# microsoft/M3P

Hardware: AMD Instinct MI355X
Metric: pre-train samples/sec (whole node), 12L/768d seq=128+36 (higher is better)
Workload: dtype bf16; 1 GPU; cfg2: 12L/768d/12h, 36 regions + 128 tokens, V=250002, 19 MLM targets/seq + ITM BCE, dropout 0.10, adam_inverse_sqrt + clip 5; per_gpu_batch=256, global_batch=256, seq_len=164, parallelism=dp1, prewarm_steps=36

## Files before the change

include/m3p_hip.h:

```cpp
#ifndef M3P_HIP_H
#define M3P_HIP_H

#include <stddef.h>
#include <stdint.h>

#ifdef __cplusplus
extern "C" {
#endif

#define M3P_API __attribute__((visibility("default")))

#define M3P_OK 0
#define M3P_EINVAL (-1)
#define M3P_ENOTIMPL (-2)
#define M3P_ENOMEM (-3)

M3P_API const char* m3p_version(void);


enum {
  M3P_EPI_NONE = 0,
  M3P_EPI_BIAS = 1,
  M3P_EPI_BIAS_GELU = 2,
  M3P_EPI_BIAS_DROP_RES = 3,
// ... 96 lines not shown
M3P_API int m3p_attn_causal_fwd(const void* qkv, int ld_qkv, void* ctx, float* lse, int B, int T, int H, int dh,
                                uint32_t seed, uint32_t thresh24, float inv_keep, void* stream);
M3P_API int m3p_attn_causal_bwd(const void* qkv, int ld_qkv, const void* dctx, const float* lse, void* dqkv, int ld_dqkv,
                                int B, int T, int H, int dh, float qscale, uint32_t seed, uint32_t thresh24,
                                float inv_keep, void* stream);


M3P_API int m3p_cast_f32_bf16(const float* src, void* dst, long long n, void* stream);

M3P_API int m3p_embed_assemble_fwd(const int64_t* tok, const void* emb_bf16, const float* pos,
                                   const void* img_proj, const float* loc, const float* w_loc,
                                   const float* b_loc, const float* g_img, const float* be_img,
                                   const float* g_emb, const float* be_emb, const int32_t* totlen,
                                   void* h, void* z, float* mean_emb, float* rstd_emb, void* e,
                                   float* mean_img, float* rstd_img, int B, int T, int R, int d,
                                   uint32_t seed_img, uint32_t seed_emb, uint32_t thresh24, float inv_keep,
                                   const void* img_rows, void* stream);

M3P_API int m3p_embed_image_rows_fwd(const void* img_proj, const float* loc, const float* w_loc, const float* b_loc,
                                     const float* g_img, const float* be_img, void* e, float* mean_img,
                                     float* rstd_img, void* img_rows, int B, int R, int d, uint32_t seed_img,
                                     uint32_t thresh24, float inv_keep, void* stream);

M3P_API int m3p_embed_assemble_bwd(const void* dh, const void* z, const float* mean_emb, const float* rstd_emb,
                                   const float* g_emb, const void* e, const float* mean_img,
                                   const float* rstd_img, const float* g_img, const int64_t* tok,
                                   const int32_t* totlen, const float* loc, void* dz_scratch, void* de,
                                   float* d_g_emb, float* d_be_emb, float* d_pos, float* d_emb,
                                   void* d_tok_rows, float* d_g_img, float* d_be_img, float* d_b_img, float* d_b_loc,
                                   float* d_w_loc, int B, int T, int R, int d, int pad_index,
                                   uint32_t seed_img, uint32_t seed_emb, uint32_t thresh24, float inv_keep,
                                   int phase, void* stream);


M3P_API int m3p_gather_rows(const void* src, const int32_t* idx, void* dst, int n, int d, void* stream);
M3P_API int m3p_place_rows(const void* src, const int32_t* inv, void* dst, int rows, int d, int n, uint32_t fill_bits,
                           void* stream);
M3P_API int m3p_scatter_add_rows(const void* src, const int32_t* idx, void* dst, int n, int d, void* stream);
M3P_API int m3p_scatter_add_token_rows(const void* rows, int ld_rows, const int64_t* ids, float* dst, int n, int d,
                                       int pad_index, void* stream);

M3P_API int m3p_itm_score_fwd(const void* pre, const float* w2, const float* b2, float* pooled, float* scores, int B,
                              int d, void* stream);
M3P_API int m3p_itm_score_bwd(const float* dscores, const float* pooled, const float* w2, void* dpre16, void* dpreT16,
                              int ldt, float* db1, float* dw2, float* db2, int B, int d, void* stream);

M3P_API int m3p_ce_fwd_bwd(void* logits, int ld, int n_rows, int V, const int64_t* target, float* row_loss,
                           float* loss_sum, float loss_scale, float grad_scale, void* stream);

M3P_API int m3p_ce_lse_from_blocks(const void* stats, int n_blocks, int n_rows, const void* logits, int ld, const int64_t* target,
                                   float* row_loss, float* row_lse, void* scratch, void* stream);
M3P_API int m3p_ce_bwd_colsum(void* logits, int ld, int n_rows, int V, const int64_t* target, const float* row_lse,
                              float grad_scale, float* colsum, void* workspace, size_t workspace_bytes, void* stream);
M3P_API size_t m3p_ce_colsum_workspace_bytes(int ld, int n_rows);
M3P_API int m3p_ce_fwd_bwd_colsum(void* logits, int ld, int n_rows, int V, const int64_t* target, float* row_loss,
                                  float* row_lse, float grad_scale, float* colsum, void* workspace,
                                  size_t workspace_bytes, void* stream);

M3P_API int m3p_ce_shift_target(const void* h, const void* emb, const float* bias, const int64_t* target, float* row_t, void* row_ref,
                                int n_rows, int d, void* stream);
M3P_API int m3p_ce_shift_rows(const void* stats, int n_blocks, int n_rows, float grad_scale, float* row_loss, float* row_s,
                              float* row_q, void* scratch, void* stream);
M3P_API int m3p_ce_shift_colsum(const void* e, int ld, int n_rows, const float* row_s, float* colsum, void* workspace,
                                size_t workspace_bytes, void* stream);
M3P_API int m3p_ce_shift_scale_rows(const void* h, const float* row_s, const float* g, void* out, int n_rows, int d, void* stream);
M3P_API int m3p_ce_shift_target_rows(const void* h, const int64_t* target, const float* row_q, const float* g, float* demb, float* dbias,
// ... 90 lines not shown
```

m3p_amd/csrc/embed.hip:

```cpp
#include "common.hpp"
#include <hip/amd_detail/amd_hip_unsafe_atomics.h>

namespace {

constexpr int EMB_BWD_BLOCKS = 512;

constexpr float kEps = 1e-12f;

template <int NI>
__device__ __forceinline__ void row_ln(const f32x4 (&v)[NI], int nchunk, int lane, float inv_d, float& mu, float& rs) {
  float s = 0.f;
#pragma unroll
  for (int i = 0; i < NI; ++i) s += (v[i][0] + v[i][1]) + (v[i][2] + v[i][3]);
  mu = wave_sum(s) * inv_d;
  float q = 0.f;
#pragma unroll
  for (int i = 0; i < NI; ++i) {
    if (lane + 64 * i < nchunk) {
      const f32x4 t = v[i] - mu;
      q += (t[0] * t[0] + t[1] * t[1]) + (t[2] * t[2] + t[3] * t[3]);
    }
  }
  rs = 1.0f / sqrtf(wave_sum(q) * inv_d + kEps);
}
// ... 284 lines not shown
        Vec4<bf16>::store(a.de + ri * d + 4 * c, ob);
        acc_e[i] += ob;
#pragma unroll
        for (int k = 0; k < 5; ++k) acc_w[k][i] += ob * lc[k];
      }
    }
  }
  block_reduce_atomic<NI>(red, acc_g, a.d_g_img, d, lane, wib);
  block_reduce_atomic<NI>(red, acc_b, a.d_be_img, d, lane, wib);
#pragma unroll
  for (int i = 0; i < NI; ++i)
#pragma unroll
    for (int j = 0; j < 4; ++j) red[wib][4 * (lane + 64 * i) + j] = acc_e[i][j];
  __syncthreads();
  for (int c = threadIdx.x; c < d; c += blockDim.x) {
    const float v = (red[0][c] + red[1][c]) + (red[2][c] + red[3][c]);
    unsafeAtomicAdd(a.d_b_img + c, v);
    unsafeAtomicAdd(a.d_b_loc + c, v);
  }
  __syncthreads();
#pragma unroll
  for (int k = 0; k < 5; ++k) {
#pragma unroll
    for (int i = 0; i < NI; ++i)
#pragma unroll
      for (int j = 0; j < 4; ++j) red[wib][4 * (lane + 64 * i) + j] = acc_w[k][i][j];
    __syncthreads();
    for (int c = threadIdx.x; c < d; c += blockDim.x)
      unsafeAtomicAdd(a.d_w_loc + (size_t)c * 5 + k, (red[0][c] + red[1][c]) + (red[2][c] + red[3][c]));
    __syncthreads();
  }
}

__global__ __launch_bounds__(256) void cast_f32_bf16_kernel(const float* __restrict__ src, bf16* __restrict__ dst, size_t n4) {
  for (size_t i = (size_t)blockIdx.x * blockDim.x + threadIdx.x; i < n4; i += (size_t)gridDim.x * blockDim.x)
    Vec4<bf16>::store(dst + 4 * i, Vec4<float>::load(src + 4 * i));
}

inline int ni_of(int d) { return (d + 255) / 256; }

int launch_embed_fwd(const EmbedFwdArgs& a, void* stream);
}

extern "C" {

int m3p_cast_f32_bf16(const float* src, void* dst, long long n, void* stream) {
  if (n <= 0 || (n % 4) != 0 || ((uintptr_t)src & 15) || ((uintptr_t)dst & 7)) return M3P_EINVAL;
  const size_t n4 = (size_t)n / 4;
  const int blocks = (int)((n4 + 255) / 256 < 4096 ? (n4 + 255) / 256 : 4096);
  hipLaunchKernelGGL(cast_f32_bf16_kernel, dim3(blocks), dim3(256), 0, (hipStream_t)stream, src, (bf16*)dst, n4);
  M3P_CHECK_LAUNCH();
  return M3P_OK;
}

int m3p_embed_assemble_fwd(const int64_t* tok, const void* emb_bf16, const float* pos, const void* img_proj,
                           const float* loc, const float* w_loc, const float* b_loc, const float* g_img,
                           const float* be_img, const float* g_emb, const float* be_emb, const int32_t* totlen,
                           void* h, void* z, float* mean_emb, float* rstd_emb, void* e, float* mean_img,
                           float* rstd_img, int B, int T, int R, int d, uint32_t seed_img, uint32_t seed_emb,
                           uint32_t thresh24, float inv_keep, const void* img_rows, void* stream) {
  if (B <= 0 || T < 0 || R < 0 || d <= 0 || (d % 4) != 0 || d > 1024) return M3P_EINVAL;
  if (img_rows && ((uintptr_t)img_rows & 7)) return M3P_EINVAL;
  EmbedFwdArgs a = {tok, (const bf16*)emb_bf16, pos, (const bf16*)img_proj, loc, w_loc, b_loc, g_img, be_img, g_emb, be_emb,
                    totlen, (bf16*)h, (bf16*)z, mean_emb, rstd_emb, (bf16*)e, mean_img, rstd_img, B, T, R, d,
                    seed_img, seed_emb, thresh24, inv_keep, (bf16*)const_cast<void*>(img_rows), img_rows ? 2 : 0};
  return launch_embed_fwd(a, stream);
}

int m3p_embed_image_rows_fwd(const void* img_proj, const float* loc, const float* w_loc, const float* b_loc,
                             const float* g_img, const float* be_img, void* e, float* mean_img, float* rstd_img,
                             void* img_rows, int B, int R, int d, uint32_t seed_img, uint32_t thresh24, float inv_keep,
                             void* stream) {
  if (B <= 0 || R <= 0 || d <= 0 || (d % 4) != 0 || d > 1024 || !img_rows || ((uintptr_t)img_rows & 7)) return M3P_EINVAL;
  EmbedFwdArgs a = {nullptr, nullptr, nullptr, (const bf16*)img_proj, loc, w_loc, b_loc, g_img, be_img, nullptr, nullptr,
                    nullptr, nullptr, nullptr, nullptr, nullptr, (bf16*)e, mean_img, rstd_img, B, 0, R, d,
                    seed_img, 0u, thresh24, inv_keep, (bf16*)img_rows, 1};
  return launch_embed_fwd(a, stream);
}

}

namespace {
int launch_embed_fwd(const EmbedFwdArgs& a, void* stream) {
  const int B = a.B, T = a.T, R = a.R, d = a.d;
  const int rows = B * (R + T);
  const int blocks = (rows + 3) / 4 < 4096 ? (rows + 3) / 4 : 4096;
  hipStream_t st = (hipStream_t)stream;
  switch (ni_of(d)) {
    case 1: hipLaunchKernelGGL(embed_fwd_kernel<1>, dim3(blocks), dim3(256), 0, st, a); break;
    case 2: hipLaunchKernelGGL(embed_fwd_kernel<2>, dim3(blocks), dim3(256), 0, st, a); break;
    case 3: hipLaunchKernelGGL(embed_fwd_kernel<3>, dim3(blocks), dim3(256), 0, st, a); break;
    default: hipLaunchKernelGGL(embed_fwd_kernel<4>, dim3(blocks), dim3(256), 0, st, a); break;
  }
  M3P_CHECK_LAUNCH();
  return M3P_OK;
}
}

extern "C" {

int m3p_embed_assemble_bwd(const void* dh, const void* z, const float* mean_emb, const float* rstd_emb,
                           const float* g_emb, const void* e, const float* mean_img, const float* rstd_img,
                           const float* g_img, const int64_t* tok, const int32_t* totlen, const float* loc,
                           void* dz_scratch, void* de, float* d_g_emb, float* d_be_emb, float* d_pos, float* d_emb,
                           void* d_tok_rows, float* d_g_img, float* d_be_img, float* d_b_img, float* d_b_loc, float* d_w_loc,
                           int B, int T, int R, int d, int pad_index, uint32_t seed_img, uint32_t seed_emb,
                           uint32_t thresh24, float inv_keep, int phase, void* stream) {
  if (B <= 0 || T < 0 || R < 0 || d <= 0 || (d % 4) != 0 || d > 1024 || phase < 0 || phase > 2) return M3P_EINVAL;
  int bsplit = 1;
  while (bsplit < 16 && (R + T) * bsplit < EMB_BWD_BLOCKS && B / (4 * bsplit) >= 8) bsplit *= 2;
  EmbedBwdArgs a = {(const bf16*)dh, (const bf16*)z, mean_emb, rstd_emb, g_emb, (const bf16*)e, mean_img, rstd_img, g_img,
                    tok, totlen, loc, (bf16*)dz_scratch, (bf16*)de, d_g_emb, d_be_emb, d_pos, d_emb,
                    (bf16*)d_tok_rows, d_g_img, d_be_img, d_b_img, d_b_loc, d_w_loc, B, T, R, d, pad_index, bsplit,
                    seed_img, seed_emb, thresh24, inv_keep};
  hipStream_t st = (hipStream_t)stream;
  const int S = R + T;
#define M3P_EMB_BWD(NI)                                                                              \
  do {                                                                                               \
    if (phase != 2) hipLaunchKernelGGL(embed_bwd_rows_kernel<NI>, dim3(S* bsplit), dim3(256), 0, st, a);             \
    if (R > 0 && phase != 1) hipLaunchKernelGGL(embed_bwd_img_kernel<NI>, dim3(R* bsplit), dim3(256), 0, st, a);   \
  } while (0)
  switch (ni_of(d)) {
    case 1: M3P_EMB_BWD(1); break;
    case 2: M3P_EMB_BWD(2); break;
    case 3: M3P_EMB_BWD(3); break;
    default: M3P_EMB_BWD(4); break;
  }
#undef M3P_EMB_BWD
  M3P_CHECK_LAUNCH();
  return M3P_OK;
}

}
```

m3p_amd/csrc/glue.hip:

```cpp
#include "common.hpp"

namespace {

__global__ __launch_bounds__(256)
void seq_masks_kernel(const long long* __restrict__ len_a, const long long* __restrict__ len_b, int B, int S,
                      int* __restrict__ totlen, uint8_t* __restrict__ rowmask) {
  const int b = blockIdx.x;
  const int n = (int)(len_a[b] + (len_b ? len_b[b] : 0));
  if (threadIdx.x == 0) totlen[b] = n;
  for (int s = threadIdx.x; s < S; s += blockDim.x) rowmask[(size_t)b * S + s] = (s < n) ? 1 : 0;
}

__global__ __launch_bounds__(1024)
void mask_to_rows_kernel(const uint8_t* __restrict__ mask, int n_mask, int inner, long long s0, long long s1,
                         long long soff, int d, int* __restrict__ rows, int n_rows) {
  __shared__ int wsum[16];
  __shared__ int total_sh;
  const int tid = threadIdx.x, lane = tid & 63, w = tid >> 6;
  const int per = (n_mask + 1023) / 1024;
  const int lo = min(tid * per, n_mask), hi = min(lo + per, n_mask);
  int cnt = 0;
  for (int i = lo; i < hi; ++i) cnt += mask[i] ? 1 : 0;
  int inc = cnt;
#pragma unroll
  for (int o = 1; o < 64; o <<= 1) {
    const int v = __shfl_up(inc, o, 64);
    if (lane >= o) inc += v;
  }
  if (lane == 63) wsum[w] = inc;
  __syncthreads();
  if (tid == 0) {
    int run = 0;
    for (int i = 0; i < 16; ++i) { const int v = wsum[i]; wsum[i] = run; run += v; }
    total_sh = run;
  }
  __syncthreads();
  int pos = wsum[w] + inc - cnt;
  for (int i = lo; i < hi; ++i) {
    if (mask[i]) {
      if (pos < n_rows) {
        const int t = i / inner, b = i - t * inner;
        rows[pos] = (int)((soff + t * s0 + b * s1) / d);
      }
      ++pos;
    }
  }
  for (int k = total_sh + tid; k < n_rows; k += 1024) rows[k] = 0;
}

__global__ __launch_bounds__(256)
void cast_rows_kernel(const float* __restrict__ in, long long s0, long long s1, int n1, int cols,
                      bf16* __restrict__ out, long long nrows) {
  const int cpr = cols >> 2;
  const long long total = nrows * cpr;
  for (long long i = (long long)blockIdx.x * blockDim.x + threadIdx.x; i < total; i += (long long)gridDim.x * blockDim.x) {
    const long long row = i / cpr;
    const int c = (int)(i - row * cpr) * 4;
    const long long i0 = row / n1, i1 = row - i0 * n1;
    const f32x4 v = *reinterpret_cast<const f32x4*>(in + i0 * s0 + i1 * s1 + c);
    *reinterpret_cast<bf16x4*>(out + row * cols + c) = bf16x4{(bf16)v[0], (bf16)v[1], (bf16)v[2], (bf16)v[3]};
  }
}

template <typename TI>
__global__ __launch_bounds__(256)
void scale_to_bf16_kernel(const TI* __restrict__ in, const float* __restrict__ g, bf16* __restrict__ out, long long n4) {
  const float s = g[0];
  for (long long i = (long long)blockIdx.x * blockDim.x + threadIdx.x; i < n4; i += (long long)gridDim.x * blockDim.x) {
    f32x4 v = Vec4<TI>::load(in + 4 * i);
    v *= s;
    Vec4<bf16>::store(out + 4 * i, v);
  }
}

__global__ __launch_bounds__(256)
void axpy_dev_kernel(float* __restrict__ dst, const float* __restrict__ src, const float* __restrict__ g, long long n) {
  const float s = g[0];
  for (long long i = (long long)blockIdx.x * blockDim.x + threadIdx.x; i < n; i += (long long)gridDim.x * blockDim.x)
    dst[i] += s * src[i];
// ... 112 lines not shown
```

m3p_amd/lib.py:

```python
import ctypes as C
import os

import torch

_HERE = os.path.dirname(os.path.abspath(__file__))
LIB_PATH = os.environ.get('M3P_HIP_LIB') or os.path.join(_HERE, 'libm3p_hip.so')

EPI_NONE, EPI_BIAS, EPI_BIAS_GELU, EPI_BIAS_DROP_RES, EPI_RES, EPI_DGELU, EPI_MUL, EPI_MULQ, EPI_BIAS_GELUQ, EPI_BIAS_LSE = range(10)
KERN_NT_SKINNY, KERN_NT_W8, KERN_NT_W8_QUEUE, KERN_NT_W4, KERN_NT_RING, KERN_NT_128 = range(1, 7)
KERN_WGRAD_W4_CHUNKS, KERN_WGRAD_W4_TILES, KERN_WGRAD_RING, KERN_WGRAD_128 = range(10, 14)


class M3PError(RuntimeError):
    pass


class Epilogue(C.Structure):
    _fields_ = [
        ('bias', C.c_void_p), ('aux', C.c_void_p), ('out2', C.c_void_p), ('colsum', C.c_void_p),
        ('ld_aux', C.c_int32), ('ld_out2', C.c_int32), ('scale_cols', C.c_int32), ('scale', C.c_float),
        ('alpha', C.c_float), ('seed', C.c_uint32), ('thresh24', C.c_uint32), ('inv_keep', C.c_float),
        ('descale_a', C.c_void_p), ('descale_b', C.c_void_p),
        ('out8', C.c_void_p), ('scale8', C.c_void_p), ('amax8', C.c_void_p), ('ld_out8', C.c_int32), ('out8_bf8', C.c_int32),
        ('rng_rows', C.c_void_p),
        ('row_ref', C.c_void_p),
    ]


_p, _i, _f, _u32 = C.c_void_p, C.c_int, C.c_float, C.c_uint32

SIGNATURES = {
    'm3p_version': (C.c_char_p, []),
    'm3p_gemm_nt_bf16': (_i, [_p, _i, _p, _i, _p, _i, _i, _i, _i, _i, C.POINTER(Epilogue), _p]),
    'm3p_gemm_nt_fp8': (_i, [_p, _i, _i, _p, _i, _p, _i, _i, _i, _i, _i, C.POINTER(Epilogue), _p]),
    'm3p_quant_fp8': (_i, [_p, _i, _p, _i, _i, _i, _p, _p, _i, _p]),
    'm3p_quant_fp8_batch': (_i, [_p, _i, _i, _p]),
    'm3p_gemm_nt_streamk_f32': (_i, [_p, _i, _p, _i, _p, _i, _i, _i, _i, _f, _p]),
    'm3p_gemm_nn_streamk_f32': (_i, [_p, _i, _p, _i, _i, _p, _i, _i, _i, _i, _f, _p]),
    'm3p_gemm_nn_w4_f32': (_i, [_p, _i, _p, _i, _p, _i, _i, _i, _i, _f, _p, C.c_size_t, _p]),
    'm3p_gemm_wgrad_workspace_bytes': (C.c_size_t, []),
    'm3p_gemm_wgrad_bf16': (_i, [_p, _i, _p, _i, _p, _i, _i, _i, _i, _f, _p, C.c_size_t, _p]),
    'm3p_gemm_wgrad_store_bf16': (_i, [_p, _i, _p, _i, _p, _i, _i, _i, _i, _f, _p, C.c_size_t, _p]),
    'm3p_gemm_wgrad_pair_bf16': (_i, [_p, _i, _p, _i, _p, _i, _i, _i, _p, _i, _p, _i, _p, _i, _i, _i, _i, _f, _p, C.c_size_t, _p]),
    'm3p_layernorm_fwd': (_i, [_p, _p, _p, _p, _p, _p, _p, _i, _i, _f, _p]),
    'm3p_layernorm_bwd': (_i, [_p, _p, _p, _p, _p, _p, _p, _p, _p, _p, _p, _p, _i, _i, _u32, _u32, _f, _p]),
    'm3p_layernorm_bwd_rows': (_i, [_p, _p, _p, _p, _p, _p, _p, _p, _p, _p, _p, _p, _i, _i, _u32, _u32, _f, _p, _p]),
    'm3p_attn_fwd': (_i, [_p, _p, _p, _p, _p, _i, _i, _i, _i, _u32, _u32, _f, _p]),
    'm3p_attn_bwd': (_i, [_p, _p, _p, _p, _p, _p, _p, _p, _i, _i, _i, _i, _f, _u32, _u32, _f, _p]),
    'm3p_attn_query_fwd': (_i, [_p, _i, _p, C.c_longlong, _i, _p, _p, _i, _i, _i, _i, _i, _i, _i, _p]),
    'm3p_attn_rows_fwd': (_i, [_p, _i, _p, C.c_longlong, _i, _p, _p, _p, _i, _i, _i, _i, _i, _i, _i, _u32, _u32, _f, _p]),
    'm3p_attn_rows_bwd': (_i, [_p, _i, _p, C.c_longlong, _i, _p, _p, _p, _p, _i, _p, _i, _i, _i, _i, _i, _i, _i, _f, _u32, _u32, _f, _p]),
    'm3p_attn_causal_fwd': (_i, [_p, _i, _p, _p, _i, _i, _i, _i, _u32, _u32, _f, _p]),
    'm3p_attn_causal_bwd': (_i, [_p, _i, _p, _p, _p, _i, _i, _i, _i, _i, _f, _u32, _u32, _f, _p]),
    'm3p_cast_f32_bf16': (_i, [_p, _p, C.c_longlong, _p]),
    'm3p_embed_assemble_fwd': (_i, [_p] * 19 + [_i, _i, _i, _i, _u32, _u32, _u32, _f, _p, _p]),
    'm3p_embed_image_rows_fwd': (_i, [_p] * 10 + [_i, _i, _i, _u32, _u32, _f, _p]),
    'm3p_embed_assemble_bwd': (_i, [_p] * 24 + [_i, _i, _i, _i, _i, _u32, _u32, _u32, _f, _i, _p]),
    'm3p_dropout_rows': (_i, [_p, _i, _p, _i, _p, _i, _i, _i, _u32, _u32, _u32, _u32, _f, _p]),
    'm3p_glu_fwd': (_i, [_p, _i, _p, _i, _i, _p]),
    'm3p_glu_bwd': (_i, [_p, _i, _p, _p, _i, _i, _p]),
    'm3p_gather_rows': (_i, [_p, _p, _p, _i, _i, _p]),
    'm3p_place_rows': (_i, [_p, _p, _p, _i, _i, _i, _u32, _p]),
    'm3p_scatter_add_rows': (_i, [_p, _p, _p, _i, _i, _p]),
    'm3p_scatter_add_token_rows': (_i, [_p, _i, _p, _p, _i, _i, _i, _p]),
    'm3p_ce_fwd_bwd': (_i, [_p, _i, _i, _i, _p, _p, _p, _f, _f, _p]),
    'm3p_ce_colsum_workspace_bytes': (C.c_size_t, [_i, _i]),
    'm3p_ce_fwd_bwd_colsum': (_i, [_p, _i, _i, _i, _p, _p, _p, _f, _p, _p, C.c_size_t, _p]),
    'm3p_ce_lse_from_blocks': (_i, [_p, _i, _i, _p, _i, _p, _p, _p, _p, _p]),
    'm3p_ce_bwd_colsum': (_i, [_p, _i, _i, _i, _p, _p, _f, _p, _p, C.c_size_t, _p]),
    'm3p_ce_shift_target': (_i, [_p, _p, _p, _p, _p, _p, _i, _i, _p]),
    'm3p_ce_shift_rows': (_i, [_p, _i, _i, _f, _p, _p, _p, _p, _p]),
    'm3p_ce_shift_colsum': (_i, [_p, _i, _i, _p, _p, _p, C.c_size_t, _p]),
    'm3p_ce_shift_scale_rows': (_i, [_p, _p, _p, _p, _i, _i, _p]),
    'm3p_ce_shift_target_rows': (_i, [_p, _p, _p, _p, _p, _p, _i, _i, _p]),
    'm3p_ce_shift_dh': (_i, [_p, _p, _p, _p, _p, _p, _p, _i, _i, _p]),
    'm3p_ce_eval': (_i, [_p, _i, _i, _i, _p, _p, _p, _p]),
    'm3p_colsum_bf16': (_i, [_p, _i, _i, _i, _p, _p, _p]),
    'm3p_sumsq_f32': (_i, [_p, C.c_longlong, _p, _p]),
    'm3p_sumsq_ranges_f32': (_i, [_p, _p, _p, _i, _p, _p]),
    'm3p_adam_step': (_i, [_p, _p, _p, _p, _p, C.c_longlong, _f, _f, _f, _f, _f, _f, _p, _f, _f, _i, _p]),
    'm3p_adam_step_ranges': (_i, [_p, _p, _p, _p, _p, _p, _p, _p, _p, _i, _f, _f, _f, _f, _f, _p, _f, _f, _p]),
    'm3p_itm_score_fwd': (_i, [_p, _p, _p, _p, _p, _i, _i, _p]),
    'm3p_itm_score_bwd': (_i, [_p, _p, _p, _p, _p, _i, _p, _p, _p, _i, _i, _p]),
    'm3p_gelu_bwd': (_i, [_p, _p, _p, C.c_longlong, _p]),
    'm3p_mse_fwd_bwd': (_i, [_p, _i, _p, _i, _p, _p, _i, _i, _f, _p]),
    'm3p_gelu_fwd': (_i, [_p, _p, _p, C.c_longlong, _p]),
    'm3p_gelu_fwd_gq': (_i, [_p, _p, _p, _i, _i, _p]),
    'm3p_gelu_fwd_q8': (_i, [_p, _p, _p, C.c_longlong, _p, _p, _p]),
    'm3p_transpose_batch_bf16': (_i, [_p, _i, _i, _p]),
    'm3p_transpose_bf16': (_i, [_p, _p, _i, _i, _i, _i, _p]),
# ... 63 lines not shown
```

m3p_amd/ops.py:

```python
import ctypes as C
import os

import torch

from . import lib as L

BF16 = torch.bfloat16
_DEBUG_CHECKS = os.environ.get('M3P_DEBUG_CHECKS') == '1'

PROFILE = None
_EPI_NAMES = ['gemm_nt/none', 'gemm_nt/bias', 'gemm_nt/bias_gelu', 'gemm_nt/bias_drop_res', 'gemm_nt/res',
              'gemm_nt/dgelu', 'gemm_nt/mul', 'gemm_nt/mulq', 'gemm_nt/bias_geluq', 'gemm_nt/bias_lse']


PROFILE_ONLY = None


def _prof_begin(key=None):
    if PROFILE is None or (PROFILE_ONLY is not None and key != PROFILE_ONLY):
        return None
    e = torch.cuda.Event(enable_timing=True)
    e.record()
    return e

# ... 444 lines not shown
    mean_e = torch.empty(B * S, dtype=torch.float32, device=dev)
    rstd_e = torch.empty(B * S, dtype=torch.float32, device=dev)
    if img_rows is not None:
        assert img_rows.dtype == BF16 and img_rows.is_contiguous() and img_rows.shape == (B * R, d)
        e, mean_i, rstd_i = img_saved
    else:
        e = torch.empty((max(R * B, 1), d), dtype=BF16, device=dev)
        mean_i = torch.empty(max(R * B, 1), dtype=torch.float32, device=dev)
        rstd_i = torch.empty(max(R * B, 1), dtype=torch.float32, device=dev)
    th, ik = _drop_args(p_drop)
    rc = L.load().m3p_embed_assemble_fwd(
        tok.data_ptr(), emb16.data_ptr(), pos.data_ptr(), L.ptr(img_proj), L.ptr(loc), w_loc.data_ptr(),
        b_loc.data_ptr(), g_img.data_ptr(), be_img.data_ptr(), g_emb.data_ptr(), be_emb.data_ptr(), totlen.data_ptr(),
        h.data_ptr(), z.data_ptr(), mean_e.data_ptr(), rstd_e.data_ptr(), e.data_ptr(), mean_i.data_ptr(),
        rstd_i.data_ptr(), B, T, R, d, seed_img, seed_emb, th, ik, L.ptr(img_rows), L.stream())
    L.check(rc, 'm3p_embed_assemble_fwd')
    return h, (z, mean_e, rstd_e, e, mean_i, rstd_i)


def embed_image_rows_fwd(img_proj, loc, w_loc, b_loc, g_img, be_img, B, R, d, seed_img=0, p_drop=0.0):
    dev = img_proj.device
    e = torch.empty((R * B, d), dtype=BF16, device=dev)
    mean_i = torch.empty(R * B, dtype=torch.float32, device=dev)
    rstd_i = torch.empty(R * B, dtype=torch.float32, device=dev)
    rows = torch.empty((B * R, d), dtype=BF16, device=dev)
    th, ik = _drop_args(p_drop)
    rc = L.load().m3p_embed_image_rows_fwd(img_proj.data_ptr(), loc.data_ptr(), w_loc.data_ptr(), b_loc.data_ptr(),
                                           g_img.data_ptr(), be_img.data_ptr(), e.data_ptr(), mean_i.data_ptr(),
                                           rstd_i.data_ptr(), rows.data_ptr(), B, R, d, seed_img, th, ik, L.stream())
    L.check(rc, 'm3p_embed_image_rows_fwd')
    return rows, (e, mean_i, rstd_i)


def embed_image_rows_bwd(d_rows, img_saved, g_img, loc, totlen, grads, B, R, d, seed_img=0, p_drop=0.0):
    e, mean_i, rstd_i = img_saved
    assert d_rows.dtype == BF16 and d_rows.is_contiguous() and d_rows.shape == (B * R, d)
    de = torch.empty_like(e)
    th, ik = _drop_args(p_drop)
    dummy = d_rows.data_ptr()
    args = (dummy, dummy, mean_i.data_ptr(), rstd_i.data_ptr(), g_img.data_ptr(), e.data_ptr(), mean_i.data_ptr(),
            rstd_i.data_ptr(), g_img.data_ptr(), dummy, totlen.data_ptr(), loc.data_ptr(), d_rows.data_ptr(), de.data_ptr(),
            grads['d_g_img'].data_ptr(), grads['d_be_img'].data_ptr(), grads['d_g_img'].data_ptr(), grads['d_g_img'].data_ptr(),
            None, grads['d_g_img'].data_ptr(), grads['d_be_img'].data_ptr(), grads['d_b_img'].data_ptr(),
            grads['d_b_loc'].data_ptr(), grads['d_w_loc'].data_ptr(), B, 0, R, d, -1, seed_img, 0, th, ik)
    L.check(L.load().m3p_embed_assemble_bwd(*args, 2, L.stream()), 'm3p_embed_assemble_bwd')
    return de


def embed_assemble_bwd(dh, saved, g_emb, g_img, tok, totlen, loc, grads, B, T, R, d, pad_index,
                       seed_img=0, seed_emb=0, p_drop=0.0, img_rows_bwd=None, tok_rows=None):
    z, mean_e, rstd_e, e, mean_i, rstd_i = saved
    dz = torch.empty_like(z)
    de = torch.empty_like(e)
    th, ik = _drop_args(p_drop)
    if tok_rows is not None:
        assert tok_rows.dtype == BF16 and tok_rows.is_contiguous() and tok_rows.shape == (T * B, d)
    args = (dh.data_ptr(), z.data_ptr(), mean_e.data_ptr(), rstd_e.data_ptr(), g_emb.data_ptr(), e.data_ptr(),
            mean_i.data_ptr(), rstd_i.data_ptr(), g_img.data_ptr(), tok.data_ptr(), totlen.data_ptr(), L.ptr(loc),
            dz.data_ptr(), de.data_ptr(), grads['d_g_emb'].data_ptr(), grads['d_be_emb'].data_ptr(),
            grads['d_pos'].data_ptr(), grads['d_emb'].data_ptr(), L.ptr(tok_rows), grads['d_g_img'].data_ptr(),
            grads['d_be_img'].data_ptr(), grads['d_b_img'].data_ptr(), grads['d_b_loc'].data_ptr(),
            grads['d_w_loc'].data_ptr(), B, T, R, d, pad_index, seed_img, seed_emb, th, ik)
    if img_rows_bwd is not None:
        L.check(L.load().m3p_embed_assemble_bwd(*args, 1, L.stream()), 'm3p_embed_assemble_bwd')
        dz_img = dz.view(B, R + T, d)[:, :R, :]
        dz_img.copy_(img_rows_bwd(dz_img.contiguous().view(B * R, d)).view(B, R, d))
# ... 337 lines not shown
```

Before: 8028 sequences/s.

## Add half-wave-per-row embedding fwd/bwd kernels for d=768/1024 and vectorize mask scan

Adds specialised embedding forward and backward kernels for wide hidden sizes. Each half-wave (32 lanes) owns one row, with 8-element bf16 vector loads and next-row prefetch. Blocks are assigned per sequence position with a CU-based split, so per-column parameters (pos, gamma/beta, loc weights) stay in registers or shared memory and column reductions go through shared memory. Separately, the mask-to-rows kernel now scans the mask 16 bytes at a time with bit tricks and popcount instead of a byte loop. A grid-query API is added. The cost is more code paths and more register pressure.

Result: no change. 8026 sequences/s (median of 2 runs) (-0.0%).

```diff
diff --git a/include/m3p_hip.h b/include/m3p_hip.h
--- a/include/m3p_hip.h
+++ b/include/m3p_hip.h
@@ -152,6 +152,8 @@
                                    uint32_t seed_img, uint32_t seed_emb, uint32_t thresh24, float inv_keep,
                                    int phase, void* stream);
 
+M3P_API int m3p_embed_grid_query(int B, int T, int R, int d, int* blocks);
+
 
 M3P_API int m3p_gather_rows(const void* src, const int32_t* idx, void* dst, int n, int d, void* stream);
 M3P_API int m3p_place_rows(const void* src, const int32_t* inv, void* dst, int rows, int d, int n, uint32_t fill_bits,
diff --git a/m3p_amd/csrc/embed.hip b/m3p_amd/csrc/embed.hip
--- a/m3p_amd/csrc/embed.hip
+++ b/m3p_amd/csrc/embed.hip
@@ -340,12 +340,440 @@
   }
 }
 
+__device__ __forceinline__ float half_sum(float v) {
+#pragma unroll
+  for (int o = 16; o > 0; o >>= 1) v += __shfl_xor(v, o, 64);
+  return v;
+}
+
+template <int NC>
+__device__ __forceinline__ void load_cols(const float* __restrict__ p, int sub, float (&o)[NC][8]) {
+#pragma unroll
+  for (int i = 0; i < NC; ++i) {
+    const int c = (sub + 32 * i) * 8;
+    const f32x4 lo = Vec4<float>::load(p + c), hi = Vec4<float>::load(p + c + 4);
+#pragma unroll
+    for (int e = 0; e < 4; ++e) { o[i][e] = lo[e]; o[i][4 + e] = hi[e]; }
+  }
+}
+
+template <int NC>
+__device__ __forceinline__ void load_row(const bf16* __restrict__ p, int sub, bf16x8 (&o)[NC]) {
+#pragma unroll
+  for (int i = 0; i < NC; ++i) o[i] = *reinterpret_cast<const bf16x8*>(p + (sub + 32 * i) * 8);
+}
+
+template <int NC>
+__device__ __forceinline__ void zero_row(bf16x8 (&o)[NC]) {
+#pragma unroll
+  for (int i = 0; i < NC; ++i)
+#pragma unroll
+    for (int e = 0; e < 8; ++e) o[i][e] = (bf16)0.f;
+}
+
+template <int NC>
+__device__ __forceinline__ void row_ln_hw(const float (&v)[NC][8], float inv_d, float& mu, float& rs) {
+  float s = 0.f;
+#pragma unroll
+  for (int i = 0; i < NC; ++i) s += ((v[i][0] + v[i][1]) + (v[i][2] + v[i][3])) + ((v[i][4] + v[i][5]) + (v[i][6] + v[i][7]));
+  mu = half_sum(s) * inv_d;
+  float q = 0.f;
+#pragma unroll
+  for (int i = 0; i < NC; ++i) {
+    float t[8];
+#pragma unroll
+    for (int e = 0; e < 8; ++e) { t[e] = v[i][e] - mu; t[e] *= t[e]; }
+    q += ((t[0] + t[1]) + (t[2] + t[3])) + ((t[4] + t[5]) + (t[6] + t[7]));
+  }
+  rs = 1.0f / sqrtf(half_sum(q) * inv_d + kEps);
+}
+
+__device__ __forceinline__ void drop8(float (&o)[8], uint32_t base, uint32_t seed, uint32_t thresh24, float inv_keep) {
+  if (thresh24) {
+    bool kp[8];
+    m3p_keep_even<8>(base, seed, thresh24, kp);
+#pragma unroll
+    for (int e = 0; e < 8; ++e) o[e] = kp[e] ? o[e] * inv_keep : 0.f;
+  }
+}
+
+__device__ __forceinline__ void store8(bf16* p, const float (&o)[8]) {
+  bf16x8 w;
+#pragma unroll
+  for (int e = 0; e < 8; ++e) w[e] = (bf16)o[e];
+  *reinterpret_cast<bf16x8*>(p) = w;
+}
+
+template <int NC>
+__global__ __launch_bounds__(256) void embed_fwd_hw_kernel(EmbedFwdArgs a, int fsplit) {
+  constexpr int D = 256 * NC;
+  __shared__ float par[8][D];
+  const int sub = threadIdx.x & 31, hw = threadIdx.x >> 5;
+  const int S = a.R + a.T;
+  const int s = blockIdx.x / fsplit, part = blockIdx.x - s * fsplit;
+  const int kind = s >= a.R ? 0 : (a.img_mode == 2 ? 2 : 1);
+  const float inv_d = 1.0f / (float)D;
+  float g[NC][8], be[NC][8], ps[NC][8];
+  if (a.img_mode != 1) {
+    load_cols<NC>(a.g_emb, sub, g);
+    load_cols<NC>(a.be_emb, sub, be);
+    load_cols<NC>(a.pos + (size_t)s * D, sub, ps);
+  } else {
+#pragma unroll
+    for (int i = 0; i < NC; ++i)
+#pragma unroll
+      for (int e = 0; e < 8; ++e) g[i][e] = be[i][e] = ps[i][e] = 0.f;
+  }
+  if (kind == 1) {
+    for (int j = threadIdx.x; j < D; j += 256) {
+#pragma unroll
+      for (int k = 0; k < 5; ++k) par[k][j] = a.w_loc[(size_t)j * 5 + k];
+      par[5][j] = a.b_loc[j]; par[6][j] = a.g_img[j]; par[7][j] = a.be_img[j];
+    }
+    __syncthreads();
+  }
+  const int step = 8 * fsplit;
+  const int64_t* tokrow = kind == 0 ? a.tok + (size_t)(s - a.R) * a.B : nullptr;
+  auto src_of = [&](int b, int64_t id) -> const bf16* {
+    if (kind == 0) return a.emb + (size_t)id * D;
+    if (kind == 1) return a.img_proj + ((size_t)s * a.B + b) * D;
+    return a.img_rows + ((size_t)b * a.R + s) * D;
+  };
+  int b = part * 8 + hw;
+  bf16x8 raw[NC];
+  float lc[5] = {0.f, 0.f, 0.f, 0.f, 0.f};
+  int tl = 0;
+  int64_t id_n = 0;
+  zero_row<NC>(raw);
+  if (b < a.B) {
+    load_row<NC>(src_of(b, kind == 0 ? tokrow[b] : 0), sub, raw);
+    if (kind == 1) {
+#pragma unroll
+      for (int k = 0; k < 5; ++k) lc[k] = a.loc[((size_t)s * a.B + b) * 5 + k];
+    }
+    if (a.img_mode != 1) tl = a.totlen[b];
+    if (kind == 0 && b + step < a.B) id_n = tokrow[b + step];
+  }
+  for (; b < a.B; b += step) {
+    const int bn = b + step;
+    bf16x8 raw_n[NC];
+    float lc_n[5] = {0.f, 0.f, 0.f, 0.f, 0.f};
+    int tl_n = 0;
+    zero_row<NC>(raw_n);
+    if (bn < a.B) {
+      load_row<NC>(src_of(bn, id_n), sub, raw_n);
+      if (kind == 1) {
+#pragma unroll
+        for (int k = 0; k < 5; ++k) lc_n[k] = a.loc[((size_t)s * a.B + bn) * 5 + k];
+      }
+      if (a.img_mode != 1) tl_n = a.totlen[bn];
+      if (kind == 0 && bn + step < a.B) id_n = tokrow[bn + step];
+    }
+    const size_t m = (size_t)b * S + s;
+    float v[NC][8];
+    float mu, rs;
+    if (kind == 1) {
+      const size_t ri = (size_t)s * a.B + b;
+#pragma unroll
+      for (int i = 0; i < NC; ++i) {
+        const int c = (sub + 32 * i) * 8;
+#pragma unroll
+        for (int e = 0; e < 8; ++e) {
+          float t = (float)raw[i][e] + par[5][c + e];
+          t += par[0][c + e] * lc[0] + par[1][c + e] * lc[1] + par[2][c + e] * lc[2] + par[3][c + e] * lc[3] + par[4][c + e] * lc[4];
+          v[i][e] = (float)(bf16)t;
+        }
+        store8(a.e + ri * D + c, v[i]);
+      }
+      row_ln_hw<NC>(v, inv_d, mu, rs);
+      if (sub == 0) { a.mean_img[ri] = mu; a.rstd_img[ri] = rs; }
+#pragma unroll
+      for (int i = 0; i < NC; ++i) {
+        const int c = (sub + 32 * i) * 8;
+#pragma unroll
+        for (int e = 0; e < 8; ++e) v[i][e] = (v[i][e] - mu) * rs * par[6][c + e] + par[7][c + e];
+        drop8(v[i], (uint32_t)ri * (uint32_t)D + (uint32_t)c, a.seed_img, a.thresh24, a.inv_keep);
+        if (a.img_mode == 1) store8(a.img_rows + ((size_t)b * a.R + s) * D + c, v[i]);
+      }
+    } else {
+#pragma unroll
+      for (int i = 0; i < NC; ++i)
+#pragma unroll
+        for (int e = 0; e < 8; ++e) v[i][e] = (float)raw[i][e];
+    }
+    if (a.img_mode != 1) {
+      const float mk = (s < tl) ? 1.f : 0.f;
+#pragma unroll
+      for (int i = 0; i < NC; ++i) {
+        const int c = (sub + 32 * i) * 8;
+#pragma unroll
+        for (int e = 0; e < 8; ++e) v[i][e] = (float)(bf16)((v[i][e] + ps[i][e]) * mk);
+        store8(a.z + m * D + c, v[i]);
+      }
+      row_ln_hw<NC>(v, inv_d, mu, rs);
+      if (sub == 0) { a.mean_emb[m] = mu; a.rstd_emb[m] = rs; }
+#pragma unroll
+      for (int i = 0; i < NC; ++i) {
+        const int c = (sub + 32 * i) * 8;
+        float o[8];
+#pragma unroll
+        for (int e = 0; e < 8; ++e) o[e] = (v[i][e] - mu) * rs * g[i][e] + be[i][e];
+        drop8(o, (uint32_t)m * (uint32_t)D + (uint32_t)c, a.seed_emb, a.thresh24, a.inv_keep);
+        store8(a.h + m * D + c, o);
+      }
+    }
+#pragma unroll
+    for (int i = 0; i < NC; ++i) raw[i] = raw_n[i];
+#pragma unroll
+    for (int k = 0; k < 5; ++k) lc[k] = lc_n[k];
+    tl = tl_n;
+  }
+}
+
+template <int NC>
+__device__ __forceinline__ void block_cols(float (*red)[256 * NC], const float (&acc)[NC][8], int sub, int hw) {
+#pragma unroll
+  for (int i = 0; i < NC; ++i) {
+    const int c = (sub + 32 * i) * 8;
+#pragma unroll
+    for (int e = 0; e < 8; ++e) red[hw][c + e] = acc[i][e];
+  }
+  __syncthreads();
+}
+template <int NC>
+__device__ __forceinline__ float col_of(float (*red)[256 * NC], int c) {
+  return ((red[0][c] + red[1][c]) + (red[2][c] + red[3][c])) + ((red[4][c] + red[5][c]) + (red[6][c] + red[7][c]));
+}
+
+template <int NC>
+__global__ __launch_bounds__(256) void embed_bwd_rows_hw_kernel(EmbedBwdArgs a) {
+  constexpr int D = 256 * NC;
+  __shared__ float red[8][D];
+  const int sub = threadIdx.x & 31, hw = threadIdx.x >> 5, lane = threadIdx.x & 63;
+  const int S = a.R + a.T;
+  const float inv_d = 1.0f / (float)D;
+  const int s = blockIdx.x / a.bsplit, part = blockIdx.x - s * a.bsplit;
+  const bool tokrow = s >= a.R;
+  const int64_t* toks = tokrow ? a.tok + (size_t)(s - a.R) * a.B : nullptr;
+  float g[NC][8], acc_g[NC][8], acc_b[NC][8], acc_p[NC][8];
+  load_cols<NC>(a.g_emb, sub, g);
+#pragma unroll
+  for (int i = 0; i < NC; ++i)
+#pragma unroll
+    for (int e = 0; e < 8; ++e) acc_g[i][e] = acc_b[i][e] = acc_p[i][e] = 0.f;
+  const int step = 8 * a.bsplit;
+  int b = part * 8 + hw;
+  bf16x8 rdy[NC], rz[NC];
+  float mu = 0.f, rs = 0.f;
+  int tl = 0;
+  int64_t id = -1;
+  zero_row<NC>(rdy); zero_row<NC>(rz);
+  if (b < a.B) {
+    const size_t m = (size_t)b * S + s;
+    load_row<NC>(a.dh + m * D, sub, rdy);
+    load_row<NC>(a.z + m * D, sub, rz);
+    mu = a.mean_emb[m]; rs = a.rstd_emb[m]; tl = a.totlen[b];
+    if (tokrow) id = toks[b];
+  }
+  for (; b - (hw & 1) < a.B; b += step) {
+    const bool act = b < a.B;
+    const int bn = b + step;
+    bf16x8 rdy_n[NC], rz_n[NC];
+    float mu_n = 0.f, rs_n = 0.f;
+    int tl_n = 0;
+    int64_t id_n = -1;
+    zero_row<NC>(rdy_n); zero_row<NC>(rz_n);
+    if (bn < a.B) {
+      const size_t mn = (size_t)bn * S + s;
+      load_row<NC>(a.dh + mn * D, sub, rdy_n);
+      load_row<NC>(a.z + mn * D, sub, rz_n);
+      mu_n = a.mean_emb[mn]; rs_n = a.rstd_emb[mn]; tl_n = a.totlen[bn];
+      if (tokrow) id_n = toks[bn];
+    }
+    const size_t m = (size_t)b * S + s;
+    float dy[NC][8], xh[NC][8];
+    float s1 = 0.f, s2 = 0.f;
+#pragma unroll
+    for (int i = 0; i < NC; ++i) {
+      const int c = (sub + 32 * i) * 8;
+#pragma unroll
+      for (int e = 0; e < 8; ++e) dy[i][e] = (float)rdy[i][e];
+      drop8(dy[i], (uint32_t)m * (uint32_t)D + (uint32_t)c, a.seed_emb, a.thresh24, a.inv_keep);
+#pragma unroll
+      for (int e = 0; e < 8; ++e) {
+        const float xe = ((float)rz[i][e] - mu) * rs;
+        xh[i][e] = xe;
+        const float gd = dy[i][e] * g[i][e];
+        s1 += gd; s2 += gd * xe;
+        acc_g[i][e] += dy[i][e] * xe;
+        acc_b[i][e] += dy[i][e];
+      }
+    }
+    const float c1 = half_sum(s1) * inv_d, c2 = half_sum(s2) * inv_d;
+    const float mk = (s < tl) ? 1.f : 0.f;
+    const bool live = act && id != a.pad_index && mk != 0.f;
+#pragma unroll
+    for (int i = 0; i < NC; ++i) {
+      const int c = (sub + 32 * i) * 8;
+      float o[8];
+#pragma unroll
+      for (int e = 0; e < 8; ++e) {
+        o[e] = (dy[i][e] * g[i][e] - c1 - xh[i][e] * c2) * rs * mk;
+        acc_p[i][e] += o[e];
+      }
+      if (!tokrow) {
+        if (act) store8(a.dz + m * D + c, o);
+      } else if (a.d_tok_rows) {
+        if (!live) {
+#pragma unroll
+          for (int e = 0; e < 8; ++e) o[e] = 0.f;
+        }
+        if (act) store8(a.d_tok_rows + ((size_t)(s - a.R) * a.B + b) * D + c, o);
+      } else {
+        *reinterpret_cast<f32x4*>(&red[hw][c]) = f32x4{o[0], o[1], o[2], o[3]};
+        *reinterpret_cast<f32x4*>(&red[hw][c + 4]) = f32x4{o[4], o[5], o[6], o[7]};
+      }
+    }
+    if (tokrow && !a.d_tok_rows) {
+      __builtin_amdgcn_wave_barrier();
+#pragma unroll
+      for (int r = 0; r < 2; ++r) {
+        const long long rid = __shfl((long long)id, 32 * r, 64);
+        const int rlive = __shfl((int)live, 32 * r, 64);
+        if (rlive) {
+          float* de = a.d_emb + (size_t)rid * D;
+          const float* row = red[(hw & ~1) + r];
+#pragma unroll
+          for (int k = 0; k < D / 64; ++k) unsafeAtomicAdd(de + lane + 64 * k, row[lane + 64 * k]);
+        }
+      }
+      __builtin_amdgcn_wave_barrier();
+    }
+#pragma unroll
+    for (int i = 0; i < NC; ++i) { rdy[i] = rdy_n[i]; rz[i] = rz_n[i]; }
+    mu = mu_n; rs = rs_n; tl = tl_n; id = id_n;
+  }
+  __syncthreads();
+  block_cols<NC>(red, acc_g, sub, hw);
+  for (int c = threadIdx.x; c < D; c += 256) unsafeAtomicAdd(a.d_g_emb + c, col_of<NC>(red, c));
+  __syncthreads();
+  block_cols<NC>(red, acc_b, sub, hw);
+  for (int c = threadIdx.x; c < D; c += 256) unsafeAtomicAdd(a.d_be_emb + c, col_of<NC>(red, c));
+  __syncthreads();
+  block_cols<NC>(red, acc_p, sub, hw);
+  for (int c = threadIdx.x; c < D; c += 256) unsafeAtomicAdd(a.d_pos + (size_t)s * D + c, col_of<NC>(red, c));
+}
+
+template <int NC>
+__global__ __launch_bounds__(256) void embed_bwd_img_hw_kernel(EmbedBwdArgs a, int isplit) {
+  constexpr int D = 256 * NC;
+  __shared__ float red[8][D];
+  __shared__ float wl[D * 5];
+  const int sub = threadIdx.x & 31, hw = threadIdx.x >> 5;
+  const int S = a.R + a.T;
+  const float inv_d = 1.0f / (float)D;
+  const int r = blockIdx.x / isplit, part = blockIdx.x - r * isplit;
+  float g[NC][8], acc_g[NC][8], acc_b[NC][8], acc_e[NC][8], acc_w[5][NC][8];
+  load_cols<NC>(a.g_img, sub, g);
+#pragma unroll
+  for (int i = 0; i < NC; ++i)
+#pragma unroll
+    for (int e = 0; e < 8; ++e) {
+      acc_g[i][e] = acc_b[i][e] = acc_e[i][e] = 0.f;
+#pragma unroll
+      for (int k = 0; k < 5; ++k) acc_w[k][i][e] = 0.f;
+    }
+  const int step = 8 * isplit;
+  for (int b = part * 8 + hw; b < a.B; b += step) {
+    const size_t m = (size_t)b * S + r;
+    const size_t ri = (size_t)r * a.B + b;
+    bf16x8 rdy[NC], rx[NC];
+    load_row<NC>(a.dz + m * D, sub, rdy);
+    load_row<NC>(a.e + ri * D, sub, rx);
+    const float mu = a.mean_img[ri], rs = a.rstd_img[ri];
+    float lc[5];
+#pragma unroll
+    for (int k = 0; k < 5; ++k) lc[k] = a.loc[ri * 5 + k];
+    float dy[NC][8], xh[NC][8];
+    float s1 = 0.f, s2 = 0.f;
+#pragma unroll
+    for (int i = 0; i < NC; ++i) {
+      const int c = (sub + 32 * i) * 8;
+#pragma unroll
+      for (int e = 0; e < 8; ++e) dy[i][e] = (float)rdy[i][e];
+      drop8(dy[i], (uint32_t)ri * (uint32_t)D + (uint32_t)c, a.seed_img, a.thresh24, a.inv_keep);
+#pragma unroll
+      for (int e = 0; e < 8; ++e) {
+        const float xe = ((float)rx[i][e] - mu) * rs;
+        xh[i][e] = xe;
+        const float gd = dy[i][e] * g[i][e];
+        s1 += gd; s2 += gd * xe;
+        acc_g[i][e] += dy[i][e] * xe;
+        acc_b[i][e] += dy[i][e];
+      }
+    }
+    const float c1 = half_sum(s1) * inv_d, c2 = half_sum(s2) * inv_d;
+#pragma unroll
+    for (int i = 0; i < NC; ++i) {
+      const int c = (sub + 32 * i) * 8;
+      float ob[8];
+#pragma unroll
+      for (int e = 0; e < 8; ++e) {
+        ob[e] = (float)(bf16)((dy[i][e] * g[i][e] - c1 - xh[i][e] * c2) * rs);
+        acc_e[i][e] += ob[e];
+#pragma unroll
+        for (int k = 0; k < 5; ++k) acc_w[k][i][e] += ob[e] * lc[k];
+      }
+      store8(a.de + ri * D + c, ob);
+    }
+  }
+  block_cols<NC>(red, acc_g, sub, hw);
+  for (int c = threadIdx.x; c < D; c += 256) unsafeAtomicAdd(a.d_g_img + c, col_of<NC>(red, c));
+  __syncthreads();
+  block_cols<NC>(red, acc_b, sub, hw);
+  for (int c = threadIdx.x; c < D; c += 256) unsafeAtomicAdd(a.d_be_img + c, col_of<NC>(red, c));
+  __syncthreads();
+  block_cols<NC>(red, acc_e, sub, hw);
+  for (int c = threadIdx.x; c < D; c += 256) {
+    const float v = col_of<NC>(red, c);
+    unsafeAtomicAdd(a.d_b_img + c, v);
+    unsafeAtomicAdd(a.d_b_loc + c, v);
+  }
+  __syncthreads();
+#pragma unroll
+  for (int k = 0; k < 5; ++k) {
+    block_cols<NC>(red, acc_w[k], sub, hw);
+    for (int c = threadIdx.x; c < D; c += 256) wl[c * 5 + k] = col_of<NC>(red, c);
+    __syncthreads();
+  }
+  for (int j = threadIdx.x; j < D * 5; j += 256) unsafeAtomicAdd(a.d_w_loc + j, wl[j]);
+}
+
 __global__ __launch_bounds__(256) void cast_f32_bf16_kernel(const float* __restrict__ src, bf16* __restrict__ dst, size_t n4) {
   for (size_t i = (size_t)blockIdx.x * blockDim.x + threadIdx.x; i < n4; i += (size_t)gridDim.x * blockDim.x)
     Vec4<bf16>::store(dst + 4 * i, Vec4<float>::load(src + 4 * i));
 }
 
 inline int ni_of(int d) { return (d + 255) / 256; }
+
+inline bool wide_d(int d) { return d == 768 || d == 1024; }
+template <typename... P>
+inline bool aligned16(P... p) { return (((uintptr_t)p | ...) & 15) == 0; }
+
+int num_cu() {
+  static int n = 0;
+  if (n == 0) {
+    int dev = 0, v = 0;
+    n = (hipGetDevice(&dev) == hipSuccess && hipDeviceGetAttribute(&v, hipDeviceAttributeMultiprocessorCount, dev) == hipSuccess && v > 0)
+            ? v : 256;
+  }
+  return n;
+}
+
+inline int split_for(int B, int groups, int target) {
+  const int by_rows = B / 16 > 1 ? B / 16 : 1, by_grid = (target + groups - 1) / groups;
+  return by_rows < by_grid ? by_rows : by_grid;
+}
 
 int launch_embed_fwd(const EmbedFwdArgs& a, void* stream);
 }
@@ -394,6 +822,13 @@
   const int rows = B * (R + T);
   const int blocks = (rows + 3) / 4 < 4096 ? (rows + 3) / 4 : 4096;
   hipStream_t st = (hipStream_t)stream;
+  if (wide_d(d) && aligned16(a.emb, a.img_proj, a.img_rows, a.h, a.z, a.e, a.pos, a.g_emb, a.be_emb)) {
+    const int fsplit = split_for(B, R + T, 4 * num_cu());
+    if (d == 768) hipLaunchKernelGGL(embed_fwd_hw_kernel<3>, dim3((R + T) * fsplit), dim3(256), 0, st, a, fsplit);
+    else hipLaunchKernelGGL(embed_fwd_hw_kernel<4>, dim3((R + T) * fsplit), dim3(256), 0, st, a, fsplit);
+    M3P_CHECK_LAUNCH();
+    return M3P_OK;
+  }
   switch (ni_of(d)) {
     case 1: hipLaunchKernelGGL(embed_fwd_kernel<1>, dim3(blocks), dim3(256), 0, st, a); break;
     case 2: hipLaunchKernelGGL(embed_fwd_kernel<2>, dim3(blocks), dim3(256), 0, st, a); break;
@@ -423,6 +858,20 @@
                     seed_img, seed_emb, thresh24, inv_keep};
   hipStream_t st = (hipStream_t)stream;
   const int S = R + T;
+  if (wide_d(d) && aligned16(dh, z, e, dz_scratch, de, d_tok_rows, g_emb, g_img)) {
+    a.bsplit = split_for(B, S, 2 * num_cu());
+    const int isplit = split_for(B, R > 0 ? R : 1, num_cu());
+    if (phase != 2) {
+      if (d == 768) hipLaunchKernelGGL(embed_bwd_rows_hw_kernel<3>, dim3(S * a.bsplit), dim3(256), 0, st, a);
+      else hipLaunchKernelGGL(embed_bwd_rows_hw_kernel<4>, dim3(S * a.bsplit), dim3(256), 0, st, a);
+    }
+    if (R > 0 && phase != 1) {
+      if (d == 768) hipLaunchKernelGGL(embed_bwd_img_hw_kernel<3>, dim3(R * isplit), dim3(256), 0, st, a, isplit);
+      else hipLaunchKernelGGL(embed_bwd_img_hw_kernel<4>, dim3(R * isplit), dim3(256), 0, st, a, isplit);
+    }
+    M3P_CHECK_LAUNCH();
+    return M3P_OK;
+  }
 #define M3P_EMB_BWD(NI)                                                                              \
   do {                                                                                               \
     if (phase != 2) hipLaunchKernelGGL(embed_bwd_rows_kernel<NI>, dim3(S* bsplit), dim3(256), 0, st, a);             \
@@ -439,4 +888,21 @@
   return M3P_OK;
 }
 
-}
+int m3p_embed_grid_query(int B, int T, int R, int d, int* blocks) {
+  if (B <= 0 || T < 0 || R < 0 || R + T <= 0 || d <= 0 || (d % 4) != 0 || d > 1024 || !blocks) return M3P_EINVAL;
+  const int S = R + T;
+  if (wide_d(d)) {
+    blocks[0] = S * split_for(B, S, 4 * num_cu());
+    blocks[1] = S * split_for(B, S, 2 * num_cu());
+    blocks[2] = R * split_for(B, R > 0 ? R : 1, num_cu());
+    return M3P_OK;
+  }
+  int bsplit = 1;
+  while (bsplit < 16 && S * bsplit < EMB_BWD_BLOCKS && B / (4 * bsplit) >= 8) bsplit *= 2;
+  blocks[0] = (B * S + 3) / 4 < 4096 ? (B * S + 3) / 4 : 4096;
+  blocks[1] = S * bsplit;
+  blocks[2] = R * bsplit;
+  return M3P_OK;
+}
+
+}
diff --git a/m3p_amd/csrc/glue.hip b/m3p_amd/csrc/glue.hip
--- a/m3p_amd/csrc/glue.hip
+++ b/m3p_amd/csrc/glue.hip
@@ -11,16 +11,50 @@
   for (int s = threadIdx.x; s < S; s += blockDim.x) rowmask[(size_t)b * S + s] = (s < n) ? 1 : 0;
 }
 
+__device__ __forceinline__ uint32_t nonzero_bytes(uint32_t w) {
+  return (((w & 0x7F7F7F7Fu) + 0x7F7F7F7Fu) | w) & 0x80808080u;
+}
+
+constexpr int MTR_KEEP = 8;
+
 __global__ __launch_bounds__(1024)
 void mask_to_rows_kernel(const uint8_t* __restrict__ mask, int n_mask, int inner, long long s0, long long s1,
                          long long soff, int d, int* __restrict__ rows, int n_rows) {
   __shared__ int wsum[16];
   __shared__ int total_sh;
   const int tid = threadIdx.x, lane = tid & 63, w = tid >> 6;
-  const int per = (n_mask + 1023) / 1024;
-  const int lo = min(tid * per, n_mask), hi = min(lo + per, n_mask);
+  const int head = (int)((uintptr_t)mask & 15);
+  const uint4* __restrict__ base = reinterpret_cast<const uint4*>(mask - head);
+  const int nvec = (int)(((long long)head + n_mask + 15) >> 4);
+  const int per = (nvec + 1023) / 1024;
+  const int v0 = min(tid * per, nvec), v1 = min(v0 + per, nvec);
+  auto piece = [&](int v) -> uint4 {
+    const uint4 x = base[v];
+    uint32_t f[4] = {nonzero_bytes(x.x), nonzero_bytes(x.y), nonzero_bytes(x.z), nonzero_bytes(x.w)};
+    const long long lo = (long long)v * 16 - head;
+    if (lo < 0 || lo + 16 > n_mask) {
+#pragma unroll
+      for (int j = 0; j < 4; ++j)
+#pragma unroll
+        for (int k = 0; k < 4; ++k) {
+          const long long idx = lo + 4 * j + k;
+          if (idx < 0 || idx >= n_mask) f[j] &= ~(0x80u << (8 * k));
+        }
+    }
+    return uint4{f[0], f[1], f[2], f[3]};
+  };
+  uint4 keep[MTR_KEEP];
   int cnt = 0;
-  for (int i = lo; i < hi; ++i) cnt += mask[i] ? 1 : 0;
+#pragma unroll
+  for (int k = 0; k < MTR_KEEP; ++k) {
+    keep[k] = uint4{0u, 0u, 0u, 0u};
+    if (v0 + k < v1) keep[k] = piece(v0 + k);
+    cnt += __popc(keep[k].x) + __popc(keep[k].y) + __popc(keep[k].z) + __popc(keep[k].w);
+  }
+  for (int v = v0 + MTR_KEEP; v < v1; ++v) {
+    const uint4 f = piece(v);
+    cnt += __popc(f.x) + __popc(f.y) + __popc(f.z) + __popc(f.w);
+  }
   int inc = cnt;
 #pragma unroll
   for (int o = 1; o < 64; o <<= 1) {
@@ -36,15 +70,27 @@
   }
   __syncthreads();
   int pos = wsum[w] + inc - cnt;
-  for (int i = lo; i < hi; ++i) {
-    if (mask[i]) {
-      if (pos < n_rows) {
-        const int t = i / inner, b = i - t * inner;
-        rows[pos] = (int)((soff + t * s0 + b * s1) / d);
+  auto emit = [&](int v, const uint4& f) {
+    const uint32_t fl[4] = {f.x, f.y, f.z, f.w};
+#pragma unroll
+    for (int j = 0; j < 4; ++j) {
+      uint32_t m = fl[j];
+      while (m) {
+        const int k = (__ffs(m) - 1) >> 3;
+        m &= m - 1;
+        if (pos < n_rows) {
+          const int i = v * 16 - head + 4 * j + k;
+          const int t = i / inner, b = i - t * inner;
+          rows[pos] = (int)((soff + t * s0 + b * s1) / d);
+        }
+        ++pos;
       }
-      ++pos;
-    }
-  }
+    }
+  };
+#pragma unroll
+  for (int k = 0; k < MTR_KEEP; ++k)
+    if (v0 + k < v1) emit(v0 + k, keep[k]);
+  for (int v = v0 + MTR_KEEP; v < v1; ++v) emit(v, piece(v));
   for (int k = total_sh + tid; k < n_rows; k += 1024) rows[k] = 0;
 }
 
diff --git a/m3p_amd/lib.py b/m3p_amd/lib.py
--- a/m3p_amd/lib.py
+++ b/m3p_amd/lib.py
@@ -56,6 +56,7 @@
     'm3p_embed_assemble_fwd': (_i, [_p] * 19 + [_i, _i, _i, _i, _u32, _u32, _u32, _f, _p, _p]),
     'm3p_embed_image_rows_fwd': (_i, [_p] * 10 + [_i, _i, _i, _u32, _u32, _f, _p]),
     'm3p_embed_assemble_bwd': (_i, [_p] * 24 + [_i, _i, _i, _i, _i, _u32, _u32, _u32, _f, _i, _p]),
+    'm3p_embed_grid_query': (_i, [_i, _i, _i, _i, _p]),
     'm3p_dropout_rows': (_i, [_p, _i, _p, _i, _p, _i, _i, _i, _u32, _u32, _u32, _u32, _f, _p]),
     'm3p_glu_fwd': (_i, [_p, _i, _p, _i, _i, _p]),
     'm3p_glu_bwd': (_i, [_p, _i, _p, _p, _i, _i, _p]),
diff --git a/m3p_amd/ops.py b/m3p_amd/ops.py
--- a/m3p_amd/ops.py
+++ b/m3p_amd/ops.py
@@ -500,6 +500,12 @@
     return rows, (e, mean_i, rstd_i)
 
 
+def embed_grid(B, T, R, d):
+    blocks = (C.c_int * 3)()
+    L.check(L.load().m3p_embed_grid_query(B, T, R, d, blocks), 'm3p_embed_grid_query')
+    return tuple(blocks)
+
+
 def embed_image_rows_bwd(d_rows, img_saved, g_img, loc, totlen, grads, B, R, d, seed_img=0, p_drop=0.0):
     e, mean_i, rstd_i = img_saved
     assert d_rows.dtype == BF16 and d_rows.is_contiguous() and d_rows.shape == (B * R, d)
```
